# PaddlePaddle/Paddle3D

Hardware: AMD Instinct MI355X
Metric: scenes/sec CenterPoint-Pillars nuScenes 300k-pt sweeps (higher is better)
Workload: dtype f32

## Files before the change

### include/paddle3d_amd.h

```cpp
#ifndef PADDLE3D_AMD_H
#define PADDLE3D_AMD_H

#include <stddef.h>
#include <stdint.h>

#ifdef __cplusplus
extern "C" {
#endif

#define PD3_OK 0
#define PD3_EINVAL (-1)
#define PD3_EWORKSPACE (-2)
#define PD3_EUNSUPPORTED (-3)

int pd3_version(void);
const char *pd3_target_arch(void);

int pd3_selfcheck_lds_atomic_order(const uint32_t *addr, uint32_t *old, int blocks, int waves_per_block, int rounds,
                                   int table, void *stream);

size_t pd3_hard_voxelize_workspace(int batch, int64_t max_points, int num_point_dim,
                                   const float *voxel_size, const float *point_cloud_range,
                                   int max_num_points_in_voxel, int max_voxels);
int pd3_hard_voxelize(const float *points, const int32_t *num_points, int batch, int64_t max_points,
// ... 20 lines not shown
                          int32_t *num_points_per_voxel, int32_t *num_voxels, int32_t *coors_batched,
                          void *workspace, size_t workspace_bytes, void *stream);

int pd3_dynamic_voxelize(const float *points, int64_t num_points, int num_point_dim, const float *voxel_size,
                         const float *point_cloud_range, int32_t *coors, void *stream);

size_t pd3_pointpillars_scatter_workspace(int batch, int ny, int nx);
int pd3_pointpillars_scatter(const float *voxel_features, const int32_t *coords,
                             int64_t num_pillars, int channels, int batch, int ny, int nx,
                             float *canvas, void *workspace, size_t workspace_bytes, void *stream);

int pd3_pointpillars_inverse_map(const int32_t *coords, int64_t num_pillars, int batch, int ny, int nx,
                                 int32_t *inv, void *stream);
int pd3_scatter_conv3x3_bias_relu(const float *voxel_features, const int32_t *inv, const float *w_packed,
                                  const float *bias, int batch, int cin, int cout, int ny, int nx, int stride,
                                  int relu, float *out, int out_w, void *stream);

size_t pd3_pillar_conv_rulebook_workspace(int batch, int ny, int nx, int stride);
int pd3_pillar_conv_rulebook(const int32_t *inverse_map, int batch, int ny, int nx, int stride, int32_t *nbr,
                             int32_t *out_cell, int32_t *cell_row, int32_t *n_out, int capacity, int32_t *order,
                             void *workspace, size_t workspace_bytes, void *stream);
int pd3_rows_to_dense_fill(const float *rows, const int32_t *cell_row, const float *fill, int batch, int channels, int h,
                           int w, float *out, void *stream);

int pd3_pillar_feature_net(const float *voxels, const int32_t *num_points, const int32_t *coors,
                           int64_t num_pillars, int max_points, int num_point_dim,
                           int voxel_center_dims, float vx, float vy, float vz, float x_offset,
                           float y_offset, float z_offset, const float *w1, const float *scale1,
                           const float *shift1, int c1, const float *w2, const float *scale2,
                           const float *shift2, int c2, float *out, void *stream);

int pd3_pillar_feature_net_path(const float *voxels, const int32_t *num_points, const int32_t *coors,
                                int64_t num_pillars, int max_points, int num_point_dim,
                                int voxel_center_dims, float vx, float vy, float vz, float x_offset,
                                float y_offset, float z_offset, const float *w1, const float *scale1,
                                const float *shift1, int c1, const float *w2, const float *scale2,
                                const float *shift2, int c2, float *out, int path, void *stream);

int pd3_pillar_feature_net_indexed(const float *points, int64_t points_per_frame, const int32_t *vox_span,
                                   const int32_t *point_list, int64_t list_stride, const int32_t *coors,
                                   int64_t num_pillars, int pillars_per_frame, int max_points, int num_point_dim,
                                   int voxel_center_dims, float vx, float vy, float vz, float x_offset,
                                   float y_offset, float z_offset, const float *w1, const float *scale1,
                                   const float *shift1, int c1, const float *w2, const float *scale2,
                                   const float *shift2, int c2, float *out, void *stream);

// ... 361 lines not shown
```

### paddle3d_amd/_lib.py

```python
from __future__ import annotations

import ctypes as C
import os
from functools import lru_cache

_HERE = os.path.dirname(os.path.abspath(__file__))
LIB_PATH = os.path.join(_HERE, "lib", "libpaddle3d_amd.so")

c_f32p = C.c_void_p
c_i32p = C.c_void_p

_SIGNATURES = {
    "pd3_version": (C.c_int, []),
    "pd3_target_arch": (C.c_char_p, []),
    "pd3_hard_voxelize_workspace": (C.c_size_t, [C.c_int, C.c_int64, C.c_int, C.c_void_p, C.c_void_p,
                                                 C.c_int, C.c_int]),
    "pd3_hard_voxelize": (C.c_int, [C.c_void_p, C.c_void_p, C.c_int, C.c_int64, C.c_int, C.c_void_p,
                                    C.c_void_p, C.c_int, C.c_int, C.c_void_p, C.c_void_p, C.c_void_p,
                                    C.c_void_p, C.c_void_p, C.c_void_p, C.c_size_t, C.c_void_p]),
    "pd3_hard_voxelize_f64": (C.c_int, [C.c_void_p, C.c_void_p, C.c_int, C.c_int64, C.c_int, C.c_void_p,
                                    C.c_void_p, C.c_int, C.c_int, C.c_void_p, C.c_void_p, C.c_void_p,
                                    C.c_void_p, C.c_void_p, C.c_void_p, C.c_size_t, C.c_void_p]),
    "pd3_hard_voxelize_path": (C.c_int, [C.c_void_p, C.c_void_p, C.c_int, C.c_int64, C.c_int, C.c_void_p,
                                         C.c_void_p, C.c_int, C.c_int, C.c_void_p, C.c_void_p, C.c_void_p,
# ... 242 lines not shown
_SIGNATURES_BEVFORMER = {
    "pd3_bevformer_point_sampling": (C.c_int, [C.c_void_p] * 3 + [C.c_int] * 6 + [C.c_void_p] * 5),
    "pd3_bevformer_sca": (C.c_int, [C.c_void_p] * 7 + [C.c_int] * 9 + [C.c_void_p] * 2),
    "pd3_bevformer_tsa": (C.c_int, [C.c_void_p] * 6 + [C.c_int] * 7 + [C.c_void_p] * 2),
}

SYMBOLS_BEVFORMER = tuple(_SIGNATURES_BEVFORMER)

_SIGNATURES_BEVFORMER_DEC = {
    "pd3_mha_forward": (C.c_int, [C.c_void_p] * 3 + [C.c_int] * 5 + [C.c_float] + [C.c_void_p] * 2),
    "pd3_bevformer_dec_ca": (C.c_int, [C.c_void_p] * 6 + [C.c_int] * 8 + [C.c_void_p] * 2),
    "pd3_nms_free_decode": (C.c_int, [C.c_void_p] * 3 + [C.c_int] * 5 + [C.c_double, C.c_int] + [C.c_void_p] * 5),
}

SYMBOLS_BEVFORMER_DEC = tuple(_SIGNATURES_BEVFORMER_DEC)

_SIGNATURES_PETR = {
    "pd3_mha_stream_forward": (C.c_int, [C.c_void_p] * 4 + [C.c_int] * 5 + [C.c_float] + [C.c_void_p] * 2),
    "pd3_petr_coords3d": (C.c_int, [C.c_void_p] + [C.c_int] * 6 + [C.c_double, C.c_void_p, C.c_int] + [C.c_void_p] * 4),
}

SYMBOLS_PETR = tuple(_SIGNATURES_PETR)


class Paddle3DAmdError(RuntimeError):
    pass


@lru_cache(maxsize=None)
def lib() -> C.CDLL:
    if not os.path.exists(LIB_PATH):
        raise Paddle3DAmdError(
            f"{LIB_PATH} not found: build it with `python -m paddle3d_amd.build` "
            "(there is no CPU / PyTorch fallback for the HIP ops)")
    handle = C.CDLL(LIB_PATH)
    for name, (res, args) in (list(_SIGNATURES.items()) + list(_SIGNATURES_ROI.items()) +
                              list(_SIGNATURES_HEAD.items()) + list(_SIGNATURES_PVRCNN.items()) +
                              list(_SIGNATURES_CADDN.items()) + list(_SIGNATURES_BEVFORMER.items()) +
                              list(_SIGNATURES_BEVFORMER_DEC.items()) + list(_SIGNATURES_PETR.items())):
        try:
            fn = getattr(handle, name)
        except AttributeError as e:
            raise Paddle3DAmdError(f"{LIB_PATH} does not export {name}") from e
        fn.restype = res
        fn.argtypes = args
    return handle


def check(status: int, what: str) -> None:
    if status == 0:
        return
    if status < 0:
        msg = {-1: "invalid argument", -2: "workspace too small", -3: "unsupported configuration"}.get(
            status, "error")
        raise Paddle3DAmdError(f"{what}: {msg} (status {status})")
    raise Paddle3DAmdError(f"{what}: HIP error {status}")
```

### paddle3d_amd/csrc/pillar_conv.hip

```cpp
#include "../../include/paddle3d_amd.h"
#include "common.hpp"
#include "scan.hpp"

namespace pd3 {

struct PcGrid {
  int ny, nx, ho, wo, stride, pad;
};

__device__ __forceinline__ int pc_lookup(const int* __restrict__ inv, const PcGrid& g, int b, int oy, int ox, int k) {
  const int iy = oy * g.stride - g.pad + k / 3, ix = ox * g.stride - g.pad + k % 3;
  if (iy < 0 || iy >= g.ny || ix < 0 || ix >= g.nx) return -1;
  return inv[((int64_t)b * g.ny + iy) * g.nx + ix];
}

__global__ __launch_bounds__(256) void pc_flags_kernel(const int* __restrict__ inv, PcGrid g, int64_t cells,
                                                       int* __restrict__ flags) {
  const int64_t i = (int64_t)blockIdx.x * blockDim.x + threadIdx.x;
  if (i >= cells) return;
  const int plane = g.ho * g.wo;
  const int b = (int)(i / plane), r = (int)(i - (int64_t)b * plane);
  const int oy = r / g.wo, ox = r - oy * g.wo;
  int any = 0;
#pragma unroll
  for (int k = 0; k < 9; ++k) any |= pc_lookup(inv, g, b, oy, ox, k) >= 0 ? 1 : 0;
// ... 120 lines not shown
  }
}

__global__ __launch_bounds__(256) void rows_to_dense_fill_kernel(const float* __restrict__ rows,
                                                                 const int* __restrict__ cell_row,
                                                                 const float* __restrict__ fill, int channels,
                                                                 int64_t plane, float* __restrict__ out) {
  const int b = blockIdx.z;
  const int c = blockIdx.y * 4;
  const int64_t cell0 = ((int64_t)blockIdx.x * blockDim.x + threadIdx.x) * 4;
  if (cell0 >= plane) return;
  const int4 src = *reinterpret_cast<const int4*>(cell_row + (int64_t)b * plane + cell0);
  const int id[4] = {src.x, src.y, src.z, src.w};
  const float4 f = fill ? *reinterpret_cast<const float4*>(fill + c) : make_float4(0.f, 0.f, 0.f, 0.f);
  float* o = out + ((int64_t)b * channels + c) * plane + cell0;
  float4 r[4];
#pragma unroll
  for (int k = 0; k < 4; ++k) r[k] = id[k] >= 0 ? *reinterpret_cast<const float4*>(rows + (int64_t)id[k] * channels + c) : f;
  typedef float pc_f32x4 __attribute__((ext_vector_type(4)));
  __builtin_nontemporal_store(pc_f32x4{r[0].x, r[1].x, r[2].x, r[3].x}, reinterpret_cast<pc_f32x4*>(o + 0 * plane));
  __builtin_nontemporal_store(pc_f32x4{r[0].y, r[1].y, r[2].y, r[3].y}, reinterpret_cast<pc_f32x4*>(o + 1 * plane));
  __builtin_nontemporal_store(pc_f32x4{r[0].z, r[1].z, r[2].z, r[3].z}, reinterpret_cast<pc_f32x4*>(o + 2 * plane));
  __builtin_nontemporal_store(pc_f32x4{r[0].w, r[1].w, r[2].w, r[3].w}, reinterpret_cast<pc_f32x4*>(o + 3 * plane));
}

}

using namespace pd3;

extern "C" size_t pd3_pillar_conv_rulebook_workspace(int batch, int ny, int nx, int stride) {
  if (batch <= 0 || ny <= 0 || nx <= 0 || stride <= 0) return 0;
  const int64_t cells = (int64_t)batch * ((ny + 2 - 3) / stride + 1) * ((nx + 2 - 3) / stride + 1);
  return align_up((size_t)cells * sizeof(int), 256) + align_up((size_t)scan_num_tiles(cells) * sizeof(int), 256);
}

extern "C" int pd3_pillar_conv_rulebook(const int32_t* inverse_map, int batch, int ny, int nx, int stride, int32_t* nbr,
                                        int32_t* out_cell, int32_t* cell_row, int32_t* n_out, int capacity,
                                        int32_t* order, void* workspace, size_t workspace_bytes, void* stream) {
  if (!inverse_map || !nbr || !out_cell || !cell_row || !n_out || !workspace || batch <= 0 || ny <= 0 || nx <= 0 ||
      capacity <= 0)
    return PD3_EINVAL;
  if (stride != 1 && stride != 2) return PD3_EUNSUPPORTED;
  PcGrid g{ny, nx, (ny + 2 - 3) / stride + 1, (nx + 2 - 3) / stride + 1, stride, 1};
  const int64_t cells = (int64_t)batch * g.ho * g.wo;
  if (cells >= ((int64_t)1 << 31)) return PD3_EUNSUPPORTED;
  if (workspace_bytes < pd3_pillar_conv_rulebook_workspace(batch, ny, nx, stride)) return PD3_EWORKSPACE;
// ... 6 lines not shown
  static_assert(kPcThreads >= 512 && 8192 % kPcWindow == 0, "a thread per bin; whole sub-windows per window");
  pc_rulebook_order_kernel<<<(unsigned)(ceil_div(capacity, 8192) * (8192 / kPcWindow)), kPcThreads, 0, s>>>(inverse_map, g, out_cell, n_out,
                                                                                     capacity, nbr, order);
  return launch_status();
}

extern "C" int pd3_rows_to_dense_fill(const float* rows, const int32_t* cell_row, const float* fill, int batch,
                                      int channels, int h, int w, float* out, void* stream) {
  if (!rows || !cell_row || !out || batch <= 0 || channels <= 0 || h <= 0 || w <= 0) return PD3_EINVAL;
  const int64_t plane = (int64_t)h * w;
  if (plane % 4 != 0 || channels % 4 != 0 || channels / 4 > 65535 || batch > 65535) return PD3_EUNSUPPORTED;
  if (reinterpret_cast<uintptr_t>(rows) % 16 != 0 || reinterpret_cast<uintptr_t>(out) % 16 != 0 ||
      reinterpret_cast<uintptr_t>(cell_row) % 16 != 0 || (fill && reinterpret_cast<uintptr_t>(fill) % 16 != 0))
    return PD3_EINVAL;
  if (channels % kRdCh == 0) {
    dim3 grid((unsigned)ceil_div(plane, kRdCells), (unsigned)(channels / kRdCh), (unsigned)batch);
    rows_to_dense_tile_kernel<<<grid, 256, 0, static_cast<hipStream_t>(stream)>>>(rows, cell_row, fill, channels, plane, out);
    return launch_status();
  }
  dim3 grid((unsigned)ceil_div(plane / 4, 256), (unsigned)(channels / 4), (unsigned)batch);
  rows_to_dense_fill_kernel<<<grid, 256, 0, static_cast<hipStream_t>(stream)>>>(rows, cell_row, fill, channels, plane, out);
  return launch_status();
}
```

### paddle3d_amd/csrc/sparse_conv_x3.hip

```cpp
#include "../../include/paddle3d_amd.h"
#include "common.hpp"

namespace pd3 {

typedef __bf16 sx_b8 __attribute__((ext_vector_type(8)));
typedef float sx_f32x16 __attribute__((ext_vector_type(16)));
typedef float sx_f32x4 __attribute__((ext_vector_type(4)));

constexpr int kSxRows = 256;
constexpr int kSxMaxK = 27;

struct SpGemmX3Args {
  const float* in;
  const int32_t* nbr;
  const __bf16* wpk;
  const float *bias, *scale, *shift;
  const float* residual;
  float* out;
  const int* n_out_dev;
  int n_out_cap, K, cin, cout, relu;
  const int32_t* order;
};

__device__ __forceinline__ void sx_split(const sx_f32x4 lo4, const sx_f32x4 hi4, sx_b8& h, sx_b8& m, sx_b8& l) {
#pragma unroll
  for (int e = 0; e < 8; ++e) {
    const float x = e < 4 ? lo4[e & 3] : hi4[e & 3];
    const __bf16 a = (__bf16)x;
    const float r1 = x - (float)a;
    const __bf16 b = (__bf16)r1;
    const float r2 = r1 - (float)b;
    h[e] = a;
    m[e] = b;
    l[e] = (__bf16)r2;
  }
}

template <int NC, int KC, int RB>
__global__ __launch_bounds__(64 * (8 / RB), RB == 1 ? 1 : 2) void sp_gemm_rows_x3_kernel(SpGemmX3Args a) {
  constexpr int THREADS = 64 * (8 / RB);
  constexpr int S = KC / 16;
  constexpr int COUT = NC * 32;
  constexpr int LINE = KC + 8;
  constexpr int WSZ = 3 * COUT * LINE;
  constexpr int WQ = 3 * COUT * KC / 8;
  constexpr int WPT = (WQ + THREADS - 1) / THREADS;
  extern __shared__ __attribute__((aligned(16))) unsigned char sx_smem[];
  __bf16* Ws = reinterpret_cast<__bf16*>(sx_smem);
  int* nbs = reinterpret_cast<int*>(Ws + 2 * WSZ);
  uint32_t* masks = reinterpret_cast<uint32_t*>(nbs + kSxRows * a.K);
  int* rows = reinterpret_cast<int*>(masks + 16);
  const int lane = lane_id(), wave = wave_id();
  const int l31 = lane & 31, kh = lane >> 5;
  const int K = a.K, cin = a.cin;
  const int n_out = a.n_out_dev ? min(*a.n_out_dev, a.n_out_cap) : a.n_out_cap;
  const int tile = sp_window_tile(blockIdx.x, (n_out + kSxRows - 1) / kSxRows, 8192 / kSxRows);
  if (tile < 0) return;
  const int row0 = tile * kSxRows;
  if (threadIdx.x < kSxRows) {
// ... 40 lines not shown
  for (int rb = 0; rb < RB; ++rb) {
    blk_mask[rb] = masks[1 + RB * wave + rb];
    wave_mask |= blk_mask[rb];
  }
  const int nchunks = cin / KC;

  sx_f32x16 acc[NC][RB];
#pragma unroll
  for (int i = 0; i < NC; ++i)
#pragma unroll
    for (int rb = 0; rb < RB; ++rb)
#pragma unroll
      for (int r = 0; r < 16; ++r) acc[i][rb][r] = 0.f;
  sx_b8 wreg[WPT];
  sx_b8 bpa[RB][S][3], bpb[RB == 1 ? RB : 1][RB == 1 ? S : 1][3];
  sx_f32x4 raw_a[RB][S][2], raw_b[RB][S][2];
  const sx_f32x4 fz = {0.f, 0.f, 0.f, 0.f};
#pragma unroll
  for (int rb = 0; rb < RB; ++rb)
#pragma unroll
    for (int s = 0; s < S; ++s) raw_a[rb][s][0] = raw_a[rb][s][1] = raw_b[rb][s][0] = raw_b[rb][s][1] = fz;

  auto fetch_w = [&](int k, int c) {
    const sx_b8* wk = reinterpret_cast<const sx_b8*>(a.wpk) + ((int64_t)k * nchunks + c) * WQ;
#pragma unroll
    for (int i = 0; i < WPT; ++i) {
      const int e = min((int)threadIdx.x + i * THREADS, WQ - 1);
      wreg[i] = wk[e];
    }
  };
  auto stash_w = [&](__bf16* dst) {
#pragma unroll
    for (int i = 0; i < WPT; ++i) {
      const int e = threadIdx.x + i * THREADS;
      if (WQ % THREADS != 0 && e >= WQ) break;
      const int line = e / (KC / 8), q = e - line * (KC / 8);
      *reinterpret_cast<sx_b8*>(dst + line * LINE + q * 8) = wreg[i];
    }
  };
  auto fetch_b = [&](int k, int c, sx_f32x4 (&dst)[RB][S][2], int (&jv)[RB]) {
#pragma unroll
    for (int rb = 0; rb < RB; ++rb) {
      const bool on = k >= 0 && ((blk_mask[rb] >> k) & 1u);
      const int j = on ? nbs[(wave * (32 * RB) + rb * 32 + l31) * K + k] : -1;
      jv[rb] = j;
      const sx_f32x4* src = reinterpret_cast<const sx_f32x4*>(a.in + (int64_t)max(j, 0) * cin + c * KC + kh * (KC / 2));
#pragma unroll
      for (int s = 0; s < S; ++s) {
        dst[rb][s][0] = src[2 * s];
        dst[rb][s][1] = src[2 * s + 1];
      }
    }
  };
  auto split_b = [&](int k, const sx_f32x4 (&src)[RB][S][2], const int (&jv)[RB], sx_b8 (&bcur)[RB][S][3]) {
#pragma unroll
    for (int rb = 0; rb < RB; ++rb) {
      if (!((blk_mask[rb] >> k) & 1u)) continue;
      const bool live = jv[rb] >= 0;
#pragma unroll
      for (int s = 0; s < S; ++s) {
// ... 22 lines not shown
  fetch_w(k, c);
  fetch_b(k, c, raw_a, j_a);
  fetch_b(k2, c2, raw_b, j_b);
  stash_w(Ws);
  if ((wave_mask >> k) & 1u) split_b(k, raw_a, j_a, bpa);
  __syncthreads();
  const bool cut_first = RB == 1 && wave >= 4;
  auto step = [&](sx_f32x4 (&near)[RB][S][2], int (&jn)[RB], sx_f32x4 (&far)[RB][S][2], int (&jf)[RB],
                  sx_b8 (&bcur)[RB][S][3], sx_b8 (&bnext)[RB][S][3]) {
    const bool more = k2 >= 0;
    int k3 = k2, c3 = c2;
    if (more) next_step(k3, c3);
    fetch_w(more ? k2 : k, more ? c2 : c);
    fetch_b(k3, c3, far, jf);
    const bool cut = more && ((wave_mask >> k2) & 1u);
    if (cut_first && cut) split_b(k2, near, jn, bnext);
    if ((wave_mask >> k) & 1u) {
      const __bf16* wl = Ws + buf * WSZ + l31 * LINE + kh * 8;
#pragma unroll
      for (int i = 0; i < NC; ++i) {
#pragma unroll
        for (int s = 0; s < S; ++s) {
          sx_b8 av[3];
#pragma unroll
          for (int p = 0; p < 3; ++p) av[p] = *reinterpret_cast<const sx_b8*>(wl + (p * COUT + i * 32) * LINE + s * 16);
#pragma unroll
          for (int rb = 0; rb < RB; ++rb) {
            if (!((blk_mask[rb] >> k) & 1u)) continue;
            acc[i][rb] = __builtin_amdgcn_mfma_f32_32x32x16_bf16(av[0], bcur[rb][s][2], acc[i][rb], 0, 0, 0);
            acc[i][rb] = __builtin_amdgcn_mfma_f32_32x32x16_bf16(av[2], bcur[rb][s][0], acc[i][rb], 0, 0, 0);
            acc[i][rb] = __builtin_amdgcn_mfma_f32_32x32x16_bf16(av[1], bcur[rb][s][1], acc[i][rb], 0, 0, 0);
            acc[i][rb] = __builtin_amdgcn_mfma_f32_32x32x16_bf16(av[0], bcur[rb][s][1], acc[i][rb], 0, 0, 0);
            acc[i][rb] = __builtin_amdgcn_mfma_f32_32x32x16_bf16(av[1], bcur[rb][s][0], acc[i][rb], 0, 0, 0);
            acc[i][rb] = __builtin_amdgcn_mfma_f32_32x32x16_bf16(av[0], bcur[rb][s][0], acc[i][rb], 0, 0, 0);
          }
        }
      }
    }
    stash_w(Ws + (buf ^ 1) * WSZ);
    if (!cut_first && cut) split_b(k2, near, jn, bnext);
    __syncthreads();
    buf ^= 1;
    k = k2;
    c = c2;
    k2 = k3;
    c2 = c3;
  };
  if constexpr (RB == 1) {
    while (k >= 0) {
      step(raw_b, j_b, raw_a, j_a, bpa, bpb);
      if (k < 0) break;
      step(raw_a, j_a, raw_b, j_b, bpb, bpa);
    }
  } else {
    while (k >= 0) {
      step(raw_b, j_b, raw_a, j_a, bpa, bpa);
      if (k < 0) break;
// ... 130 lines not shown
```

### paddle3d_amd/ops/conv.py

```python
from __future__ import annotations

import ctypes

import torch

from ._common import check, lib, ptr, require_gpu, stream_ptr

__all__ = ["pack_conv3x3_weight", "conv3x3_bias_relu", "supported", "pitch4", "pack_grouped_weight", "grouped_conv3x3_small",
           "grouped_small_supported", "winograd_supported", "pack_winograd_weight", "conv3x3_winograd_bias_relu",
           "patch_mode", "patch_supported", "pack_patch_weight", "patch_conv_bias_relu",
           "patch_x3_supported", "pack_patch_weight_x3", "patch_conv_x3_bias_relu", "split_bf16x3",
           "conv3x3_s2_x3_supported", "pack_conv3x3_s2_x3_weight", "conv3x3_s2_x3_bias_relu",
           "winograd43_input_transform", "conv3x3_winograd43_ppv_bias_relu",
           "winograd43_supported", "winograd43_tile", "pack_winograd43_weight", "conv3x3_winograd43_bias_relu",
           "WINOGRAD43_PP_MIN_CIN", "winograd43_pp_supported", "pack_winograd43_lane_weight", "conv3x3_winograd43_pp_bias_relu",
           "f16_supported", "f16_tile", "pack_conv3x3_f16_weight", "conv3x3_f16_bias_relu", "to_f16_nhwc",
           "pack_grouped_weight_f16", "grouped_conv3x3_small_f16", "conv3x3_f16_bias_relu_dual",
           "s2_f16_supported", "conv3x3_s2_f16_bias_relu", "scatter_conv_s2_f16_supported",
           "scatter_conv3x3_s2_f16_bias_relu", "scatter_conv_sparse_supported", "scatter_conv3x3_sparse"]


def pitch4(w: int) -> int:
    return (int(w) + 3) // 4 * 4


def supported(cin: int, cout: int, h: int, w: int, stride: int = 1) -> bool:
    return stride in (1, 2) and cin % 8 == 0 and cout % 64 == 0 and h % stride == 0 and w % stride == 0


def pack_conv3x3_weight(weight: torch.Tensor) -> torch.Tensor:
    cout, cin = weight.shape[:2]
    assert weight.shape[2:] == (3, 3) and cout % 64 == 0 and cin % 8 == 0
    w = weight.reshape(cout // 64, 64, cin // 8, 4, 2, 9).permute(0, 2, 3, 5, 4, 1)
    return w.reshape(cout // 64, cin // 8, 72, 64).contiguous()


def conv3x3_bias_relu(x: torch.Tensor, w_packed: torch.Tensor, bias, cout: int, relu: bool = True,
                      stride: int = 1, out: torch.Tensor | None = None, w_valid: int | None = None) -> torch.Tensor:
    xx = require_gpu(x, "conv3x3_bias_relu")
    n, cin, h, w = xx.shape
    wv = w if w_valid is None else int(w_valid)
    if out is None:
# ... 4 lines not shown
    return out


def scatter_conv_supported(cin: int, cout: int, ny: int, nx: int, stride: int) -> bool:
    return stride == 2 and cin % 8 == 0 and cout % 64 == 0 and ny % 2 == 0 and nx % 2 == 0


def scatter_conv3x3_bias_relu(canvas, w_packed: torch.Tensor, bias, cout: int, relu: bool = True) -> torch.Tensor:
    f, inv = canvas.features, canvas.inv
    n, cin, ny, nx = canvas.shape
    wo = pitch4(nx // 2)
    out = torch.empty((n, cout, ny // 2, wo), dtype=torch.float32, device=f.device)
    check(lib().pd3_scatter_conv3x3_bias_relu(ptr(f), ptr(inv), ptr(w_packed), ptr(bias), n, cin, cout, ny, nx, 2,
                                              int(bool(relu)), ptr(out), wo, stream_ptr(f.device)),
          "scatter_conv3x3_bias_relu")
    return out


def scatter_conv_sparse_supported(cin: int, cout: int, ny: int, nx: int, stride: int) -> bool:
    ho, wo = (ny - 1) // stride + 1, (nx - 1) // stride + 1
    return stride == 2 and cin % 16 == 0 and cout in (64, 128) and wo % 4 == 0 and (ho * wo) % 4 == 0


def scatter_conv3x3_sparse(canvas, weight: torch.Tensor, bias: torch.Tensor, packed=None, relu: bool = True):
    from . import sparse_conv3d as sp
    from ._common import workspace

    f, inv = canvas.features, canvas.inv
    n, cin, ny, nx = canvas.shape
    cout = int(weight.shape[0])
    ho, wo = (ny - 1) // 2 + 1, (nx - 1) // 2 + 1
    cap = n * ho * wo
    dev = f.device
    L = lib()
    nbr = torch.empty((cap, 9), dtype=torch.int32, device=dev)
    out_cell = torch.empty((cap,), dtype=torch.int32, device=dev)
    cell_row = torch.empty((n, ho * wo), dtype=torch.int32, device=dev)
    n_out = torch.empty((1,), dtype=torch.int32, device=dev)
    ws = workspace(L.pd3_pillar_conv_rulebook_workspace(n, ny, nx, 2), dev)
    order = torch.empty((int(L.pd3_sparse_tile_order_entries(cap)),), dtype=torch.int32, device=dev)
    check(L.pd3_pillar_conv_rulebook(ptr(inv), n, ny, nx, 2, ptr(nbr), ptr(out_cell), ptr(cell_row), ptr(n_out), cap,
                                     ptr(order), ptr(ws), ws.numel(), stream_ptr(dev)), "pillar_conv_rulebook")
    idx = sp.SparseIndices(None, nbr, cap, (1, ho, wo), 9, order, n_out)
    if packed is None:
        packed = sp.pack_weight_bf16x3(weight.permute(2, 3, 1, 0).reshape(1, 3, 3, cin, cout).contiguous())
    rows = sp.features_bf16x3(f, idx, packed, cin, cout, bias, None, None, None, relu)
    fill = torch.relu(bias) if relu else bias
    out = torch.empty((n, cout, ho, wo), dtype=torch.float32, device=dev)
    check(L.pd3_rows_to_dense_fill(ptr(rows), ptr(cell_row), ptr(fill.contiguous()), n, cout, ho, wo, ptr(out),
                                   stream_ptr(dev)), "rows_to_dense_fill")
    return out, packed


def winograd_supported(cin: int, cout: int, h: int, w: int) -> bool:
    return cin % 8 == 0 and cout % 32 == 0 and w % 4 == 0


def pack_winograd_weight(weight: torch.Tensor) -> torch.Tensor:
    cout, cin = weight.shape[:2]
    assert weight.shape[2:] == (3, 3) and cout % 32 == 0 and cin % 8 == 0
    g = torch.tensor([[1.0, 0.0, 0.0], [0.5, 0.5, 0.5], [0.5, -0.5, 0.5], [0.0, 0.0, 1.0]], dtype=torch.float64,
                     device=weight.device)
    u = torch.einsum("ij,ocjk,lk->ocil", g, weight.double(), g).float()
    u = u.reshape(cout // 32, 2, 16, cin // 8, 8, 16).permute(0, 3, 1, 4, 2, 5)
    return u.contiguous()


def conv3x3_winograd_bias_relu(x: torch.Tensor, u_packed: torch.Tensor, bias, cout: int, relu: bool = True,
                               out: torch.Tensor | None = None) -> torch.Tensor:
    xx = require_gpu(x, "conv3x3_winograd_bias_relu")
# ... 398 lines not shown
```

Before: 2393.

## Add fused tile kernel for stride-2 pillar conv and trim rows-path allocations

Adds a new kernel that computes the stride-2 3x3 pillar convolution one 8x32 output tile at a time. It gathers the neighbourhood inverse map, optionally stages pillar features in LDS, buckets pixels by neighbour mask, runs bf16x3 MFMA with double-buffered weights, and writes dense output with a bias fill. This would skip the separate rulebook, row GEMM and dense-fill passes, but the default form stays "rows", so the new kernel does not run unless a caller asks for it. The rows path gets a smaller rulebook capacity bound by pillar count and a cached relu(bias) fill, and shared helpers move into a header.

```diff
diff --git a/include/paddle3d_amd.h b/include/paddle3d_amd.h
--- a/include/paddle3d_amd.h
+++ b/include/paddle3d_amd.h
@@ -66,6 +66,9 @@
                              void *workspace, size_t workspace_bytes, void *stream);
 int pd3_rows_to_dense_fill(const float *rows, const int32_t *cell_row, const float *fill, int batch, int channels, int h,
                            int w, float *out, void *stream);
+int pd3_pillar_conv3x3_s2_tile(const float *features, const int32_t *inverse_map, const void *weight_packed,
+                               const float *bias, int relu, int batch, int cin, int cout, int ny, int nx, float *out,
+                               void *stream);
 
 int pd3_pillar_feature_net(const float *voxels, const int32_t *num_points, const int32_t *coors,
                            int64_t num_pillars, int max_points, int num_point_dim,
diff --git a/paddle3d_amd/_lib.py b/paddle3d_amd/_lib.py
--- a/paddle3d_amd/_lib.py
+++ b/paddle3d_amd/_lib.py
@@ -288,6 +288,13 @@
 
 SYMBOLS_PETR = tuple(_SIGNATURES_PETR)
 
+_SIGNATURES_PILLAR_TILE = {
+    "pd3_pillar_conv3x3_s2_tile": (C.c_int, [C.c_void_p, C.c_void_p, C.c_void_p, C.c_void_p, C.c_int, C.c_int, C.c_int,
+                                             C.c_int, C.c_int, C.c_int, C.c_void_p, C.c_void_p]),
+}
+
+SYMBOLS_PILLAR_TILE = tuple(_SIGNATURES_PILLAR_TILE)
+
 
 class Paddle3DAmdError(RuntimeError):
     pass
@@ -303,7 +310,8 @@
     for name, (res, args) in (list(_SIGNATURES.items()) + list(_SIGNATURES_ROI.items()) +
                               list(_SIGNATURES_HEAD.items()) + list(_SIGNATURES_PVRCNN.items()) +
                               list(_SIGNATURES_CADDN.items()) + list(_SIGNATURES_BEVFORMER.items()) +
-                              list(_SIGNATURES_BEVFORMER_DEC.items()) + list(_SIGNATURES_PETR.items())):
+                              list(_SIGNATURES_BEVFORMER_DEC.items()) + list(_SIGNATURES_PETR.items()) +
+                              list(_SIGNATURES_PILLAR_TILE.items())):
         try:
             fn = getattr(handle, name)
         except AttributeError as e:
diff --git a/paddle3d_amd/csrc/pillar_conv.hip b/paddle3d_amd/csrc/pillar_conv.hip
--- a/paddle3d_amd/csrc/pillar_conv.hip
+++ b/paddle3d_amd/csrc/pillar_conv.hip
@@ -1,6 +1,8 @@
 #include "../../include/paddle3d_amd.h"
 #include "common.hpp"
 #include "scan.hpp"
+#include <type_traits>
+#include "sparse_x3.hpp"
 
 namespace pd3 {
 
@@ -167,6 +169,379 @@
   __builtin_nontemporal_store(pc_f32x4{r[0].y, r[1].y, r[2].y, r[3].y}, reinterpret_cast<pc_f32x4*>(o + 1 * plane));
   __builtin_nontemporal_store(pc_f32x4{r[0].z, r[1].z, r[2].z, r[3].z}, reinterpret_cast<pc_f32x4*>(o + 2 * plane));
   __builtin_nontemporal_store(pc_f32x4{r[0].w, r[1].w, r[2].w, r[3].w}, reinterpret_cast<pc_f32x4*>(o + 3 * plane));
+}
+
+
+constexpr int kPtH = 8, kPtW = 32, kPtPix = kPtH * kPtW, kPtPH = 2 * kPtH + 1, kPtPW = 2 * kPtW + 1;
+constexpr int kPtPatch = (kPtPH * kPtPW + 3) / 4 * 4;
+constexpr int kPtCout = 64;
+constexpr int kPtTileBytes = kPtCout * kPtPix * (int)sizeof(float);
+constexpr int kPtSmall = (kPtPatch + 512 + 8 + 16) * (int)sizeof(int) + 2 * kPtPix * (int)sizeof(uint16_t);
+constexpr int kPtLds = 79872;
+constexpr int kPtMainBytes = (kPtLds - kPtSmall) / 16 * 16;
+constexpr int kPtMaxStaged = 512;
+static_assert(kPtMainBytes >= kPtTileBytes, "the output tile fits the main region");
+static_assert(kPtPix == 256, "a thread per pixel, eight 32-row blocks on four waves");
+
+struct PcTileArgs {
+  const float* in;
+  const int* inv;
+  const __bf16* wpk;
+  const float* bias;
+  float* out;
+  int cin, relu, ny, nx, ho, wo;
+};
+
+template <int KC>
+__global__ __launch_bounds__(256, 2) void pillar_conv_tile_kernel(PcTileArgs a) {
+  constexpr int NC = 2, RB = 2, THREADS = 256, COUT = kPtCout;
+  constexpr int S = KC / 16, LINE = KC + 8, WSZ = 3 * COUT * LINE, WQ = 3 * COUT * KC / 8;
+  constexpr int WPT = (WQ + THREADS - 1) / THREADS;
+  static_assert(2 * WSZ * (int)sizeof(__bf16) <= kPtTileBytes, "the staged weights live where the output tile lands");
+  extern __shared__ __attribute__((aligned(16))) unsigned char pt_smem[];
+  float* otile = reinterpret_cast<float*>(pt_smem);
+  __bf16* Ws = reinterpret_cast<__bf16*>(pt_smem);
+  float* stage = reinterpret_cast<float*>(pt_smem + 2 * WSZ * sizeof(__bf16));
+  int* patch = reinterpret_cast<int*>(pt_smem + kPtMainBytes);
+  int* hist = patch + kPtPatch;
+  int* scr = hist + 512;
+  uint32_t* masks = reinterpret_cast<uint32_t*>(scr + 8);
+  uint16_t* sorted = reinterpret_cast<uint16_t*>(masks + 16);
+  uint16_t* smask = sorted + kPtPix;
+  const int t = threadIdx.x, lane = lane_id(), wave = wave_id();
+  const int l31 = lane & 31, kh = lane >> 5;
+  const int b = blockIdx.z, oy0 = blockIdx.y * kPtH, ox0 = blockIdx.x * kPtW;
+  const int cin = a.cin;
+
+  const int rstride = cin + 4;
+  bool staged;
+  {
+    constexpr int N = (kPtPH * kPtPW + THREADS - 1) / THREADS;
+    int v[N], slot[N];
+#pragma unroll
+    for (int u = 0; u < N; ++u) {
+      const int e = t + u * THREADS;
+      const int py = e / kPtPW, px = e - py * kPtPW;
+      const int iy = 2 * oy0 - 1 + py, ix = 2 * ox0 - 1 + px;
+      const bool in = e < kPtPH * kPtPW && iy >= 0 && iy < a.ny && ix >= 0 && ix < a.nx;
+      v[u] = in ? a.inv[((int64_t)b * a.ny + iy) * a.nx + ix] : -1;
+    }
+    if (t == 0) scr[6] = 0;
+    if (t < 16) masks[t] = 0u;
+    __syncthreads();
+#pragma unroll
+    for (int u = 0; u < N; ++u) slot[u] = v[u] >= 0 ? atomicAdd(&scr[6], 1) : -1;
+    __syncthreads();
+    const int np = scr[6];
+    const int pmax = min(kPtMaxStaged, (kPtMainBytes - 2 * WSZ * (int)sizeof(__bf16)) / (int)sizeof(float) / rstride);
+    staged = np <= pmax;
+    int* ids = hist;
+#pragma unroll
+    for (int u = 0; u < N; ++u) {
+      const int e = t + u * THREADS;
+      if (e < kPtPH * kPtPW) patch[e] = staged ? slot[u] : v[u];
+      if (staged && slot[u] >= 0) ids[slot[u]] = v[u];
+    }
+    __syncthreads();
+    if (staged) {
+      const int q4 = cin / 4, total = np * q4;
+      for (int e0 = t; e0 < total; e0 += 8 * THREADS) {
+        sx_f32x4 r[8];
+#pragma unroll
+        for (int u = 0; u < 8; ++u) {
+          const int e = min(e0 + u * THREADS, total - 1);
+          const int row = e / q4, q = e - row * q4;
+          r[u] = *reinterpret_cast<const sx_f32x4*>(a.in + (int64_t)ids[row] * cin + q * 4);
+        }
+#pragma unroll
+        for (int u = 0; u < 8; ++u) {
+          const int e = e0 + u * THREADS;
+          if (e >= total) break;
+          const int row = e / q4, q = e - row * q4;
+          *reinterpret_cast<sx_f32x4*>(stage + row * rstride + q * 4) = r[u];
+        }
+      }
+      __syncthreads();
+    }
+    hist[t] = 0;
+    hist[t + THREADS] = 0;
+  }
+  __syncthreads();
+  int m = 0;
+  {
+    const int ty = t >> 5, tx = t & 31;
+    if (oy0 + ty < a.ho && ox0 + tx < a.wo) {
+#pragma unroll
+      for (int k = 0; k < 9; ++k) m |= patch[(2 * ty + k / 3) * kPtPW + 2 * tx + k % 3] >= 0 ? 1 << k : 0;
+    }
+  }
+  if (m) atomicAdd(&hist[m], 1);
+  __syncthreads();
+  int n_rows;
+  {
+    const int h0 = hist[2 * t], h1 = hist[2 * t + 1];
+    const int base = block_exclusive_scan<THREADS>(h0 + h1, scr, n_rows);
+    hist[2 * t] = base;
+    hist[2 * t + 1] = base + h0;
+  }
+  __syncthreads();
+  if (m) {
+    const int pos = atomicAdd(&hist[m], 1);
+    sorted[pos] = (uint16_t)t;
+    smask[pos] = (uint16_t)m;
+  }
+  __syncthreads();
+  typedef float pc_f32x4 __attribute__((ext_vector_type(4)));
+  auto store_tile = [&](bool from_lds) {
+#pragma unroll 4
+    for (int i = 0; i < COUT * kPtPix / 4 / THREADS; ++i) {
+      const int e = i * THREADS + t;
+      const int c = e >> 6, p4 = e & 63;
+      const int oy = oy0 + (p4 >> 3), ox = ox0 + (p4 & 7) * 4;
+      if (oy >= a.ho || ox >= a.wo) continue;
+      pc_f32x4 v;
+      if (from_lds) {
+        v = *reinterpret_cast<const pc_f32x4*>(otile + c * kPtPix + p4 * 4);
+      } else {
+        float f = a.bias ? a.bias[c] : 0.f;
+        f = a.relu ? fmaxf(f, 0.f) : f;
+        v = pc_f32x4{f, f, f, f};
+      }
+      *reinterpret_cast<pc_f32x4*>(a.out + (((int64_t)b * COUT + c) * a.ho + oy) * a.wo + ox) = v;
+    }
+  };
+  if (n_rows == 0) {
+    store_tile(false);
+    return;
+  }
+  {
+    uint32_t mm = t < n_rows ? smask[t] : 0u;
+#pragma unroll
+    for (int d = 1; d < 32; d <<= 1) mm |= (uint32_t)__shfl_xor((int)mm, d, kWave);
+    if (l31 == 0 && mm) {
+      atomicOr(&masks[1 + (t >> 5)], mm);
+      atomicOr(&masks[0], mm);
+    }
+  }
+  __syncthreads();
+  const uint32_t wg_mask = masks[0];
+  uint32_t blk_mask[RB], wave_mask = 0u;
+  int pix[RB], pbase[RB];
+#pragma unroll
+  for (int rb = 0; rb < RB; ++rb) {
+    const int blk = rb * 4 + wave;
+    blk_mask[rb] = masks[1 + blk];
+    wave_mask |= blk_mask[rb];
+    const int slot = blk * 32 + l31;
+    pix[rb] = slot < n_rows ? (int)sorted[slot] : -1;
+    const int p = max(pix[rb], 0);
+    pbase[rb] = 2 * (p >> 5) * kPtPW + 2 * (p & 31);
+  }
+  const int nchunks = cin / KC;
+
+  sx_f32x16 acc[NC][RB];
+#pragma unroll
+  for (int i = 0; i < NC; ++i)
+#pragma unroll
+    for (int rb = 0; rb < RB; ++rb)
+#pragma unroll
+      for (int r = 0; r < 16; ++r) acc[i][rb][r] = 0.f;
+  const sx_f32x4 fz = {0.f, 0.f, 0.f, 0.f};
+  auto fetch_w = [&](int k, int c, sx_b8 (&wreg)[WPT]) {
+    const sx_b8* wk = sx_weight_chunk<COUT, KC>(a.wpk, k, nchunks, c);
+#pragma unroll
+    for (int i = 0; i < WPT; ++i) {
+      const int e = min(t + i * THREADS, WQ - 1);
+      wreg[i] = wk[e];
+    }
+  };
+  auto stash_w = [&](__bf16* dst, const sx_b8 (&wreg)[WPT]) {
+#pragma unroll
+    for (int i = 0; i < WPT; ++i) {
+      const int e = t + i * THREADS;
+      if (WQ % THREADS != 0 && e >= WQ) break;
+      *reinterpret_cast<sx_b8*>(dst + sx_stash_offset<KC>(e)) = wreg[i];
+    }
+  };
+  auto pillar = [&](int k, int rb) {
+    const bool on = k >= 0 && ((blk_mask[rb] >> k) & 1u) && pix[rb] >= 0;
+    const int kk = max(k, 0);
+    return on ? patch[pbase[rb] + (kk / 3) * kPtPW + kk % 3] : -1;
+  };
+  auto fetch_b = [&](int k, int c, sx_f32x4 (&dst)[RB][S][2], int (&jv)[RB]) {
+#pragma unroll
+    for (int rb = 0; rb < RB; ++rb) {
+      const int j = pillar(k, rb);
+      jv[rb] = j;
+      const sx_f32x4* src = reinterpret_cast<const sx_f32x4*>(a.in + (int64_t)max(j, 0) * cin + c * KC + kh * (KC / 2));
+#pragma unroll
+      for (int s = 0; s < S; ++s) {
+        dst[rb][s][0] = src[2 * s];
+        dst[rb][s][1] = src[2 * s + 1];
+      }
+    }
+  };
+  auto split_b = [&](int k, const sx_f32x4 (&src)[RB][S][2], const int (&jv)[RB], sx_b8 (&bcur)[RB][S][3]) {
+#pragma unroll
+    for (int rb = 0; rb < RB; ++rb) {
+      if (!((blk_mask[rb] >> k) & 1u)) continue;
+      const bool live = jv[rb] >= 0;
+#pragma unroll
+      for (int s = 0; s < S; ++s) {
+        sx_f32x4 lo4 = src[rb][s][0], hi4 = src[rb][s][1];
+#pragma unroll
+        for (int e = 0; e < 4; ++e) {
+          lo4[e] = live ? lo4[e] : 0.f;
+          hi4[e] = live ? hi4[e] : 0.f;
+        }
+        sx_split(lo4, hi4, bcur[rb][s][0], bcur[rb][s][1], bcur[rb][s][2]);
+      }
+    }
+  };
+  auto split_staged = [&](int k, int c, sx_b8 (&bcur)[RB][S][3]) {
+#pragma unroll
+    for (int rb = 0; rb < RB; ++rb) {
+      if (!((blk_mask[rb] >> k) & 1u)) continue;
+      const int j = pillar(k, rb);
+      const bool live = j >= 0;
+      const sx_f32x4* src = reinterpret_cast<const sx_f32x4*>(stage + max(j, 0) * rstride + c * KC + kh * (KC / 2));
+#pragma unroll
+      for (int s = 0; s < S; ++s) {
+        sx_f32x4 lo4 = src[2 * s], hi4 = src[2 * s + 1];
+#pragma unroll
+        for (int e = 0; e < 4; ++e) {
+          lo4[e] = live ? lo4[e] : 0.f;
+          hi4[e] = live ? hi4[e] : 0.f;
+        }
+        sx_split(lo4, hi4, bcur[rb][s][0], bcur[rb][s][1], bcur[rb][s][2]);
+      }
+    }
+  };
+  auto next_step = [&](int& k, int& c) {
+    if (++c < nchunks) return;
+    c = 0;
+    const uint32_t rest = wg_mask >> (k + 1);
+    k = rest ? k + 1 + __builtin_ctz(rest) : -1;
+  };
+
+  auto run = [&](auto tag) {
+    constexpr bool ST = decltype(tag)::value;
+    sx_b8 wa[WPT], wb[WPT];
+    sx_b8 bpa[RB][S][3];
+    sx_f32x4 raw_a[RB][S][2], raw_b[RB][S][2];
+    int j_a[RB], j_b[RB];
+#pragma unroll
+    for (int rb = 0; rb < RB; ++rb)
+#pragma unroll
+      for (int s = 0; s < S; ++s) raw_a[rb][s][0] = raw_a[rb][s][1] = raw_b[rb][s][0] = raw_b[rb][s][1] = fz;
+    int k = __builtin_ctz(wg_mask), c = 0, buf = 0;
+    int k2 = k, c2 = c;
+    next_step(k2, c2);
+    fetch_w(k, c, wa);
+    if constexpr (ST) fetch_w(k2 >= 0 ? k2 : k, k2 >= 0 ? c2 : c, wb);
+    if constexpr (!ST) {
+      fetch_b(k, c, raw_a, j_a);
+      fetch_b(k2, c2, raw_b, j_b);
+    }
+    stash_w(Ws, wa);
+    if ((wave_mask >> k) & 1u) {
+      if constexpr (ST) split_staged(k, c, bpa);
+      else split_b(k, raw_a, j_a, bpa);
+    }
+    __syncthreads();
+    auto step = [&](sx_f32x4 (&near)[RB][S][2], int (&jn)[RB], sx_f32x4 (&far)[RB][S][2], int (&jf)[RB],
+                    sx_b8 (&wl)[WPT], sx_b8 (&ws)[WPT]) {
+      const bool more = k2 >= 0;
+      int k3 = k2, c3 = c2;
+      if (more) next_step(k3, c3);
+      if constexpr (ST) fetch_w(k3 >= 0 ? k3 : k, k3 >= 0 ? c3 : c, wl);
+      else fetch_w(more ? k2 : k, more ? c2 : c, wl);
+      if constexpr (!ST) fetch_b(k3, c3, far, jf);
+      const bool cut = more && ((wave_mask >> k2) & 1u);
+      if ((wave_mask >> k) & 1u) {
+        const __bf16* wlds = Ws + buf * WSZ + l31 * LINE + kh * 8;
+        const bool on0 = (blk_mask[0] >> k) & 1u, on1 = (blk_mask[1] >> k) & 1u;
+        static_assert(NC == 2 && RB == 2, "the interleaving below is written out for 2 x 2 accumulators");
+#pragma unroll
+        for (int s = 0; s < S; ++s) {
+          sx_b8 av0[3], av1[3];
+          sx_load_a<COUT, KC>(wlds, 0, s, av0);
+          sx_load_a<COUT, KC>(wlds, 1, s, av1);
+#define PD3_PT_PIECE(P)                                                   \
+  do {                                                                    \
+    if (on0) sx_mfma_piece<P>(av0, bpa[0][s], acc[0][0]);                 \
+    if (on0) sx_mfma_piece<P>(av1, bpa[0][s], acc[1][0]);                 \
+    if (on1) sx_mfma_piece<P>(av0, bpa[1][s], acc[0][1]);                 \
+    if (on1) sx_mfma_piece<P>(av1, bpa[1][s], acc[1][1]);                 \
+  } while (0)
+          if (on0 && on1) {
+            const bool on0 = true, on1 = true;
+            PD3_PT_PIECE(0); PD3_PT_PIECE(1); PD3_PT_PIECE(2); PD3_PT_PIECE(3); PD3_PT_PIECE(4); PD3_PT_PIECE(5);
+          } else if (on0) {
+            const bool on0 = true, on1 = false;
+            PD3_PT_PIECE(0); PD3_PT_PIECE(1); PD3_PT_PIECE(2); PD3_PT_PIECE(3); PD3_PT_PIECE(4); PD3_PT_PIECE(5);
+          } else {
+            const bool on0 = false, on1 = true;
+            PD3_PT_PIECE(0); PD3_PT_PIECE(1); PD3_PT_PIECE(2); PD3_PT_PIECE(3); PD3_PT_PIECE(4); PD3_PT_PIECE(5);
+          }
+#undef PD3_PT_PIECE
+        }
+      }
+      stash_w(Ws + (buf ^ 1) * WSZ, ST ? ws : wl);
+      if (cut) {
+        if constexpr (ST) split_staged(k2, c2, bpa);
+        else split_b(k2, near, jn, bpa);
+      }
+      __syncthreads();
+      buf ^= 1;
+      k = k2;
+      c = c2;
+      k2 = k3;
+      c2 = c3;
+    };
+    while (k >= 0) {
+      step(raw_b, j_b, raw_a, j_a, wa, wb);
+      if (k < 0) break;
+      step(raw_a, j_a, raw_b, j_b, wb, wa);
+    }
+  };
+  if (staged) run(std::true_type{});
+  else run(std::false_type{});
+#pragma unroll 4
+  for (int i = 0; i < COUT * kPtPix / 4 / THREADS; ++i) {
+    const int e = i * THREADS + t;
+    float f = a.bias ? a.bias[e >> 6] : 0.f;
+    f = a.relu ? fmaxf(f, 0.f) : f;
+    *reinterpret_cast<pc_f32x4*>(otile + e * 4) = pc_f32x4{f, f, f, f};
+  }
+  __syncthreads();
+#pragma unroll
+  for (int rb = 0; rb < RB; ++rb) {
+    if (pix[rb] < 0) continue;
+#pragma unroll
+    for (int i = 0; i < NC; ++i) {
+#pragma unroll
+      for (int q = 0; q < 4; ++q) {
+        const int co = i * 32 + 8 * q + 4 * kh;
+        float v[4];
+#pragma unroll
+        for (int e = 0; e < 4; ++e) v[e] = acc[i][rb][4 * q + e];
+        if (a.bias) {
+          const sx_f32x4 b4 = *reinterpret_cast<const sx_f32x4*>(a.bias + co);
+#pragma unroll
+          for (int e = 0; e < 4; ++e) v[e] += b4[e];
+        }
+        if (a.relu) {
+#pragma unroll
+          for (int e = 0; e < 4; ++e) v[e] = fmaxf(v[e], 0.f);
+        }
+#pragma unroll
+        for (int e = 0; e < 4; ++e) otile[(co + e) * kPtPix + pix[rb]] = v[e];
+      }
+    }
+  }
+  __syncthreads();
+  store_tile(true);
 }
 
 }
@@ -219,3 +594,31 @@
   rows_to_dense_fill_kernel<<<grid, 256, 0, static_cast<hipStream_t>(stream)>>>(rows, cell_row, fill, channels, plane, out);
   return launch_status();
 }
+
+extern "C" int pd3_pillar_conv3x3_s2_tile(const float* features, const int32_t* inverse_map, const void* weight_packed,
+                                          const float* bias, int relu, int batch, int cin, int cout, int ny, int nx,
+                                          float* out, void* stream) {
+  if (!features || !inverse_map || !weight_packed || !out || batch <= 0 || cin <= 0 || cout <= 0 || ny <= 0 || nx <= 0)
+    return PD3_EINVAL;
+  const int ho = (ny - 1) / 2 + 1, wo = (nx - 1) / 2 + 1;
+  if (cin % 16 != 0 || cout != kPtCout || wo % 4 != 0) return PD3_EUNSUPPORTED;
+  const int64_t tx = ceil_div(wo, kPtW), ty = ceil_div(ho, kPtH);
+  if (ty > 65535 || batch > 65535) return PD3_EUNSUPPORTED;
+  if (reinterpret_cast<uintptr_t>(features) % 16 != 0 || reinterpret_cast<uintptr_t>(weight_packed) % 16 != 0 ||
+      reinterpret_cast<uintptr_t>(out) % 16 != 0 || (bias && reinterpret_cast<uintptr_t>(bias) % 16 != 0))
+    return PD3_EINVAL;
+  PcTileArgs a{features, inverse_map, static_cast<const __bf16*>(weight_packed), bias, out, cin, relu ? 1 : 0, ny, nx, ho, wo};
+  const dim3 grid((unsigned)tx, (unsigned)ty, (unsigned)batch);
+  hipStream_t s = static_cast<hipStream_t>(stream);
+  hipError_t e;
+  if (cin % 32 == 0) {
+    e = pd3_max_dynamic_lds(reinterpret_cast<const void*>(pillar_conv_tile_kernel<32>), kPtLds);
+    if (e != hipSuccess) return (int)e;
+    pillar_conv_tile_kernel<32><<<grid, 256, kPtLds, s>>>(a);
+  } else {
+    e = pd3_max_dynamic_lds(reinterpret_cast<const void*>(pillar_conv_tile_kernel<16>), kPtLds);
+    if (e != hipSuccess) return (int)e;
+    pillar_conv_tile_kernel<16><<<grid, 256, kPtLds, s>>>(a);
+  }
+  return launch_status();
+}
diff --git a/paddle3d_amd/csrc/sparse_conv_x3.hip b/paddle3d_amd/csrc/sparse_conv_x3.hip
--- a/paddle3d_amd/csrc/sparse_conv_x3.hip
+++ b/paddle3d_amd/csrc/sparse_conv_x3.hip
@@ -1,11 +1,8 @@
 #include "../../include/paddle3d_amd.h"
 #include "common.hpp"
+#include "sparse_x3.hpp"
 
 namespace pd3 {
-
-typedef __bf16 sx_b8 __attribute__((ext_vector_type(8)));
-typedef float sx_f32x16 __attribute__((ext_vector_type(16)));
-typedef float sx_f32x4 __attribute__((ext_vector_type(4)));
 
 constexpr int kSxRows = 256;
 constexpr int kSxMaxK = 27;
@@ -21,20 +18,6 @@
   int n_out_cap, K, cin, cout, relu;
   const int32_t* order;
 };
-
-__device__ __forceinline__ void sx_split(const sx_f32x4 lo4, const sx_f32x4 hi4, sx_b8& h, sx_b8& m, sx_b8& l) {
-#pragma unroll
-  for (int e = 0; e < 8; ++e) {
-    const float x = e < 4 ? lo4[e & 3] : hi4[e & 3];
-    const __bf16 a = (__bf16)x;
-    const float r1 = x - (float)a;
-    const __bf16 b = (__bf16)r1;
-    const float r2 = r1 - (float)b;
-    h[e] = a;
-    m[e] = b;
-    l[e] = (__bf16)r2;
-  }
-}
 
 template <int NC, int KC, int RB>
 __global__ __launch_bounds__(64 * (8 / RB), RB == 1 ? 1 : 2) void sp_gemm_rows_x3_kernel(SpGemmX3Args a) {
@@ -121,7 +104,7 @@
     for (int s = 0; s < S; ++s) raw_a[rb][s][0] = raw_a[rb][s][1] = raw_b[rb][s][0] = raw_b[rb][s][1] = fz;
 
   auto fetch_w = [&](int k, int c) {
-    const sx_b8* wk = reinterpret_cast<const sx_b8*>(a.wpk) + ((int64_t)k * nchunks + c) * WQ;
+    const sx_b8* wk = sx_weight_chunk<COUT, KC>(a.wpk, k, nchunks, c);
 #pragma unroll
     for (int i = 0; i < WPT; ++i) {
       const int e = min((int)threadIdx.x + i * THREADS, WQ - 1);
@@ -133,8 +116,7 @@
     for (int i = 0; i < WPT; ++i) {
       const int e = threadIdx.x + i * THREADS;
       if (WQ % THREADS != 0 && e >= WQ) break;
-      const int line = e / (KC / 8), q = e - line * (KC / 8);
-      *reinterpret_cast<sx_b8*>(dst + line * LINE + q * 8) = wreg[i];
+      *reinterpret_cast<sx_b8*>(dst + sx_stash_offset<KC>(e)) = wreg[i];
     }
   };
   auto fetch_b = [&](int k, int c, sx_f32x4 (&dst)[RB][S][2], int (&jv)[RB]) {
@@ -203,17 +185,11 @@
 #pragma unroll
         for (int s = 0; s < S; ++s) {
           sx_b8 av[3];
-#pragma unroll
-          for (int p = 0; p < 3; ++p) av[p] = *reinterpret_cast<const sx_b8*>(wl + (p * COUT + i * 32) * LINE + s * 16);
+          sx_load_a<COUT, KC>(wl, i, s, av);
 #pragma unroll
           for (int rb = 0; rb < RB; ++rb) {
             if (!((blk_mask[rb] >> k) & 1u)) continue;
-            acc[i][rb] = __builtin_amdgcn_mfma_f32_32x32x16_bf16(av[0], bcur[rb][s][2], acc[i][rb], 0, 0, 0);
-            acc[i][rb] = __builtin_amdgcn_mfma_f32_32x32x16_bf16(av[2], bcur[rb][s][0], acc[i][rb], 0, 0, 0);
-            acc[i][rb] = __builtin_amdgcn_mfma_f32_32x32x16_bf16(av[1], bcur[rb][s][1], acc[i][rb], 0, 0, 0);
-            acc[i][rb] = __builtin_amdgcn_mfma_f32_32x32x16_bf16(av[0], bcur[rb][s][1], acc[i][rb], 0, 0, 0);
-            acc[i][rb] = __builtin_amdgcn_mfma_f32_32x32x16_bf16(av[1], bcur[rb][s][0], acc[i][rb], 0, 0, 0);
-            acc[i][rb] = __builtin_amdgcn_mfma_f32_32x32x16_bf16(av[0], bcur[rb][s][0], acc[i][rb], 0, 0, 0);
+            sx_mfma6(av, bcur[rb][s], acc[i][rb]);
           }
         }
       }
diff --git a/paddle3d_amd/csrc/sparse_x3.hpp b/paddle3d_amd/csrc/sparse_x3.hpp
--- /dev/null
+++ b/paddle3d_amd/csrc/sparse_x3.hpp
@@ -0,0 +1,55 @@
+#pragma once
+#include "common.hpp"
+
+namespace pd3 {
+
+typedef __bf16 sx_b8 __attribute__((ext_vector_type(8)));
+typedef float sx_f32x16 __attribute__((ext_vector_type(16)));
+typedef float sx_f32x4 __attribute__((ext_vector_type(4)));
+
+__device__ __forceinline__ void sx_split(const sx_f32x4 lo4, const sx_f32x4 hi4, sx_b8& h, sx_b8& m, sx_b8& l) {
+#pragma unroll
+  for (int e = 0; e < 8; ++e) {
+    const float x = e < 4 ? lo4[e & 3] : hi4[e & 3];
+    const __bf16 a = (__bf16)x;
+    const float r1 = x - (float)a;
+    const __bf16 b = (__bf16)r1;
+    const float r2 = r1 - (float)b;
+    h[e] = a;
+    m[e] = b;
+    l[e] = (__bf16)r2;
+  }
+}
+
+template <int P>
+__device__ __forceinline__ void sx_mfma_piece(const sx_b8 (&av)[3], const sx_b8 (&bv)[3], sx_f32x16& acc) {
+  constexpr int A[6] = {0, 2, 1, 0, 1, 0}, B[6] = {2, 0, 1, 1, 0, 0};
+  acc = __builtin_amdgcn_mfma_f32_32x32x16_bf16(av[A[P]], bv[B[P]], acc, 0, 0, 0);
+}
+__device__ __forceinline__ void sx_mfma6(const sx_b8 (&av)[3], const sx_b8 (&bv)[3], sx_f32x16& acc) {
+  sx_mfma_piece<0>(av, bv, acc);
+  sx_mfma_piece<1>(av, bv, acc);
+  sx_mfma_piece<2>(av, bv, acc);
+  sx_mfma_piece<3>(av, bv, acc);
+  sx_mfma_piece<4>(av, bv, acc);
+  sx_mfma_piece<5>(av, bv, acc);
+}
+
+template <int COUT, int KC>
+__device__ __forceinline__ const sx_b8* sx_weight_chunk(const __bf16* wpk, int k, int nchunks, int c) {
+  return reinterpret_cast<const sx_b8*>(wpk) + ((int64_t)k * nchunks + c) * (3 * COUT * KC / 8);
+}
+
+template <int KC>
+__device__ __forceinline__ int sx_stash_offset(int e) {
+  const int line = e / (KC / 8), q = e - line * (KC / 8);
+  return line * (KC + 8) + q * 8;
+}
+
+template <int COUT, int KC>
+__device__ __forceinline__ void sx_load_a(const __bf16* wl, int i, int s, sx_b8 (&av)[3]) {
+#pragma unroll
+  for (int p = 0; p < 3; ++p) av[p] = *reinterpret_cast<const sx_b8*>(wl + (p * COUT + i * 32) * (KC + 8) + s * 16);
+}
+
+}
diff --git a/paddle3d_amd/ops/conv.py b/paddle3d_amd/ops/conv.py
--- a/paddle3d_amd/ops/conv.py
+++ b/paddle3d_amd/ops/conv.py
@@ -17,7 +17,8 @@
            "f16_supported", "f16_tile", "pack_conv3x3_f16_weight", "conv3x3_f16_bias_relu", "to_f16_nhwc",
            "pack_grouped_weight_f16", "grouped_conv3x3_small_f16", "conv3x3_f16_bias_relu_dual",
            "s2_f16_supported", "conv3x3_s2_f16_bias_relu", "scatter_conv_s2_f16_supported",
-           "scatter_conv3x3_s2_f16_bias_relu", "scatter_conv_sparse_supported", "scatter_conv3x3_sparse"]
+           "scatter_conv3x3_s2_f16_bias_relu", "scatter_conv_sparse_supported", "scatter_conv_tile_supported",
+           "scatter_conv3x3_sparse"]
 
 
 def pitch4(w: int) -> int:
@@ -68,7 +69,23 @@
     return stride == 2 and cin % 16 == 0 and cout in (64, 128) and wo % 4 == 0 and (ho * wo) % 4 == 0
 
 
-def scatter_conv3x3_sparse(canvas, weight: torch.Tensor, bias: torch.Tensor, packed=None, relu: bool = True):
+def scatter_conv_tile_supported(cin: int, cout: int, ny: int, nx: int, stride: int) -> bool:
+    wo = (nx - 1) // stride + 1
+    return stride == 2 and cin % 16 == 0 and cout == 64 and wo % 4 == 0
+
+
+def _relu_bias(bias: torch.Tensor, packed: torch.Tensor) -> torch.Tensor:
+    import weakref
+
+    c = getattr(packed, "_pd3_fill", None)
+    if c is None or c[0]() is not bias or c[1] != bias._version:
+        c = (weakref.ref(bias), bias._version, torch.relu(bias).contiguous())
+        packed._pd3_fill = c
+    return c[2]
+
+
+def scatter_conv3x3_sparse(canvas, weight: torch.Tensor, bias: torch.Tensor, packed=None, relu: bool = True, *,
+                           form=None):
     from . import sparse_conv3d as sp
     from ._common import workspace
 
@@ -76,9 +93,20 @@
     n, cin, ny, nx = canvas.shape
     cout = int(weight.shape[0])
     ho, wo = (ny - 1) // 2 + 1, (nx - 1) // 2 + 1
-    cap = n * ho * wo
     dev = f.device
     L = lib()
+    if form is None:
+        form = "rows"
+    if form not in ("tile", "rows"):
+        raise ValueError(f"scatter_conv3x3_sparse: form {form!r}")
+    if form == "tile":
+        if packed is None:
+            packed = sp.pack_weight_bf16x3(weight.permute(2, 3, 1, 0).reshape(1, 3, 3, cin, cout).contiguous())
+        out = torch.empty((n, cout, ho, wo), dtype=torch.float32, device=dev)
+        check(L.pd3_pillar_conv3x3_s2_tile(ptr(f), ptr(inv), ptr(packed), ptr(bias.contiguous()), int(bool(relu)), n, cin,
+                                           cout, ny, nx, ptr(out), stream_ptr(dev)), "pillar_conv3x3_s2_tile")
+        return out, packed
+    cap = max(1, min(n * ho * wo, 4 * int(f.shape[0])))
     nbr = torch.empty((cap, 9), dtype=torch.int32, device=dev)
     out_cell = torch.empty((cap,), dtype=torch.int32, device=dev)
     cell_row = torch.empty((n, ho * wo), dtype=torch.int32, device=dev)
@@ -91,7 +119,7 @@
     if packed is None:
         packed = sp.pack_weight_bf16x3(weight.permute(2, 3, 1, 0).reshape(1, 3, 3, cin, cout).contiguous())
     rows = sp.features_bf16x3(f, idx, packed, cin, cout, bias, None, None, None, relu)
-    fill = torch.relu(bias) if relu else bias
+    fill = _relu_bias(bias, packed) if relu else bias
     out = torch.empty((n, cout, ho, wo), dtype=torch.float32, device=dev)
     check(L.pd3_rows_to_dense_fill(ptr(rows), ptr(cell_row), ptr(fill.contiguous()), n, cout, ho, wo, ptr(out),
                                    stream_ptr(dev)), "rows_to_dense_fill")
```

New measurement: 2396 (median of 6 runs). About the same (+0.1%).
